# zhiqwang/yolort

Measured on NVIDIA H100. Metric: images/sec end-to-end (letterbox->NMS), higher is better.
Workload: dtype f16

## Files before the change

yolort_b200/_C.py:

```python
import ctypes
import itertools
import math
import os
from typing import Dict, List, Optional, Sequence, Tuple

import torch

_HERE = os.path.dirname(os.path.abspath(__file__))
LIB_PATH = os.environ.get("YB_LIB_PATH") or os.path.join(_HERE, "libyolort_b200.so")

YB_U8, YB_F16, YB_BF16, YB_F32, YB_F8E4M3 = 0, 1, 2, 3, 4
YB_LAYOUT_NCHW, YB_LAYOUT_S2D16 = 0, 1
YB_OP_CONV, YB_OP_SPP_POOL, YB_OP_UPSAMPLE2X, YB_OP_ATTENTION, YB_OP_DWCONV, YB_OP_SE, YB_OP_AVGPOOL = 0, 1, 2, 3, 4, 5, 6
YB_OP_QUANTIZE = 7
YB_ACT_NONE, YB_ACT_SILU, YB_ACT_HARDSWISH, YB_ACT_LEAKY01, YB_ACT_RELU = 0, 1, 2, 3, 4
YB_CONV_FORCE_IM2COL, YB_CONV_BAND_STEM, YB_CONV_FORCE_PLANES, YB_CONV_NO_NSPLIT, YB_CONV_ONE_CTA = 1, 2, 4, 8, 16
YB_CONV_NO_TAIL_SPLIT = 64
YB_CONV_PAIR_N64 = 128
YB_CONV_NO_TEAMS = 256
YB_CONV_E4M3_F16_OUT, YB_CONV_E4M3_BF16_OUT = 16, 32
YB_CONV_KERNEL_IM2COL, YB_CONV_KERNEL_PATCH, YB_CONV_KERNEL_E4M3 = 0, 1, 2
PATCH_TILINGS = {1: "classic", 2: "wrap", 3: "stride2"}
YB_MAX_LEVELS, YB_MAX_ANCHORS = 4, 4
NMS_TV_AUTO, NMS_EXACT_PER_CLASS, NMS_OFFSET_TRICK = 0, 1, 2
# ... 425 lines not shown
                                   ctypes.c_void_p]
    L.yb_kmeans_workspace_bytes.restype = ctypes.c_size_t
    L.yb_kmeans_workspace_bytes.argtypes = [ctypes.c_int64, ctypes.c_int, ctypes.c_int]
    L.yb_kmeans.argtypes = [ctypes.c_void_p, ctypes.c_int64, ctypes.c_int, ctypes.c_int, ctypes.c_void_p, ctypes.c_double,
                            ctypes.c_int, ctypes.c_void_p, ctypes.c_void_p, ctypes.c_void_p,
                            ctypes.POINTER(ctypes.c_int32), ctypes.c_void_p, ctypes.c_size_t, ctypes.c_void_p]
    L.yb_anchor_evolve.argtypes = [ctypes.c_void_p, ctypes.c_int64, ctypes.c_int, ctypes.c_void_p, ctypes.c_void_p,
                                   ctypes.c_int, ctypes.c_double, ctypes.c_int, ctypes.c_void_p, ctypes.c_void_p,
                                   ctypes.c_void_p, ctypes.c_void_p, ctypes.c_size_t, ctypes.c_void_p]
    L.yb_v5m_match_workspace_bytes.restype = ctypes.c_size_t
    L.yb_v5m_match_workspace_bytes.argtypes = [ctypes.c_int]
    L.yb_v5m_match.argtypes = [ctypes.c_int, ctypes.c_int] + [ctypes.c_void_p] * 5 + [ctypes.c_int] + \
        [ctypes.c_void_p] * 2 + [ctypes.c_int, ctypes.c_void_p, ctypes.c_int, ctypes.c_float, ctypes.c_float, ctypes.c_int] + \
        [ctypes.c_void_p] * 5 + [ctypes.c_size_t, ctypes.c_void_p]
    L.yb_v5m_ap_workspace_bytes.restype = ctypes.c_size_t
    L.yb_v5m_ap_workspace_bytes.argtypes = [ctypes.c_int64, ctypes.c_int]
    L.yb_v5m_ap.argtypes = [ctypes.c_void_p, ctypes.c_int64, ctypes.c_int, ctypes.c_int] + [ctypes.c_void_p] * 7 + \
        [ctypes.c_size_t, ctypes.c_void_p]
    _lib = L
    return L


def check(rc: int, what: str) -> None:
    if rc != 0:
        msg = lib().yb_last_error().decode("utf-8", "replace")
        raise NativeLibraryError(f"{what} failed (status {rc}): {msg}")


def dtype_code(dt: torch.dtype) -> int:
    try:
        return {torch.uint8: YB_U8, torch.float16: YB_F16, torch.bfloat16: YB_BF16, torch.float32: YB_F32,
                torch.float8_e4m3fn: YB_F8E4M3}[dt]
    except KeyError:
        raise NativeLibraryError(f"unsupported tensor dtype {dt}") from None


def current_stream_ptr(device: torch.device) -> int:
    return torch.cuda.current_stream(device).cuda_stream


class _NoGuard:
    def __enter__(self):
        return None

    def __exit__(self, *a):
        return False


_NO_GUARD = _NoGuard()


def device_guard(device: torch.device):
    idx = device.index if device.index is not None else torch.cuda.current_device()
    if torch.cuda.current_device() == idx:
        return _NO_GUARD
    return torch.cuda.device(idx)


def require_cuda(t: torch.Tensor, what: str) -> None:
    if not t.is_cuda:
        raise NativeLibraryError(
            f"{what}: tensor lives on {t.device}; the yolort_b200 path runs on sm_90a only (no CPU fallback)")


def letterbox_geometry(sizes: Sequence[Tuple[int, int]], min_size: float, max_size: float,
                       size_divisible: int = 32, fixed_shape: Optional[Tuple[int, int]] = None):
    n = len(sizes)
    hw = (ctypes.c_int32 * (2 * n))(*[int(v) for s in sizes for v in s])
    geoms = (LetterboxGeom * n)()
    bhw = (ctypes.c_int32 * 2)()
    fs = None
    if fixed_shape is not None:
        fs = (ctypes.c_int32 * 2)(int(fixed_shape[0]), int(fixed_shape[1]))
    check(lib().yb_letterbox_geometry(n, hw, float(min_size), float(max_size), int(size_divisible), fs, geoms, bhw),
          "yb_letterbox_geometry")
    return geoms, (int(bhw[0]), int(bhw[1]))


def scale_coords_params(Hb: int, Wb: int, h: int, w: int) -> Tuple[float, float, float]:
    out = (ctypes.c_float * 3)()
    check(lib().yb_scale_coords_params(int(Hb), int(Wb), int(h), int(w), out), "yb_scale_coords_params")
    return float(out[0]), float(out[1]), float(out[2])


_u8_lut: Dict[torch.device, torch.Tensor] = {}


def u8_lut(device: torch.device) -> torch.Tensor:
    t = _u8_lut.get(device)
    if t is None:
        t = (torch.arange(256, dtype=torch.uint8) / 255.0).to(torch.float32).to(device)
        _u8_lut[device] = t
    return t


YB_SRC_CHW, YB_SRC_HWC = 0, 1


def _is_hwc_view(im: torch.Tensor) -> bool:
    _, h, w = im.shape
    return tuple(im.stride()) == (1, 3 * w, 3) and (h > 1 or w > 1)


def letterbox(images: List[torch.Tensor], geoms, Hb: int, Wb: int, fill: float, out: torch.Tensor,
              layout: int) -> torch.Tensor:
    n = len(images)
    dev = out.device
    require_cuda(out, "letterbox")
    src_dtype = images[0].dtype
    ptrs = (ctypes.c_void_p * n)()
    keep = []
    for im in images:
        require_cuda(im, "letterbox")
        if im.dtype != src_dtype:
            raise NativeLibraryError("letterbox: all images of a batch must share a dtype")
        if im.dim() != 3 or im.shape[0] != 3:
            raise ValueError(f"images is expected to be a list of 3d tensors of shape [C, H, W], but got '{im.shape}'.")
    hwc = all(_is_hwc_view(im) for im in images)
    for i, im in enumerate(images):
        if not hwc:
            im = im.contiguous()
        keep.append(im)
        ptrs[i] = im.data_ptr()
    lut = u8_lut(dev) if src_dtype == torch.uint8 else None
    with device_guard(dev):
        check(lib().yb_letterbox_strided(n, ptrs, dtype_code(src_dtype), YB_SRC_HWC if hwc else YB_SRC_CHW, geoms,
                                         int(Hb), int(Wb), float(fill), lut.data_ptr() if lut is not None else None,
                                         out.data_ptr(), dtype_code(out.dtype), int(layout), current_stream_ptr(dev)),
              "yb_letterbox")
    stream = torch.cuda.current_stream(dev)
    seen = set()
    for im in keep:
        key = im.untyped_storage().data_ptr()
        if key not in seen:
            seen.add(key)
            im.record_stream(stream)
    return out


def conv_chain_supported(op: "OpDesc") -> bool:
    return bool(lib().yb_conv_chain_supported(ctypes.byref(op)))


def conv_config(op: "OpDesc") -> dict:
    info = ConvInfo()
    check(lib().yb_conv_config(ctypes.byref(op), ctypes.byref(info)), "yb_conv_config")
    patch = info.kernel == YB_CONV_KERNEL_PATCH
    cfg = {k: int(getattr(info, k)) for k in ("block_n", "n_tiles", "weights_resident", "tiles_per_pass", "slots", "ring",
                                               "store_cols", "smem_bytes", "grid", "chained", "resident_ctas", "m_tiles",
                                               "work_items", "tail_n", "tail_tiles", "tail_split")}
    cfg["patch_kernel"] = int(patch)
    cfg["e4m3_kernel"] = int(info.kernel == YB_CONV_KERNEL_E4M3)
    cfg["store_bufs" if patch else "epilogue_groups"] = int(info.store_bufs if patch else info.groups)
    cfg["layout"] = f"{info.resident_ctas}x{info.groups}"
    cfg["consumer_groups"] = int(info.groups)
    cfg["ctas_per_sm"] = 2 if cfg["layout"] == "2x2" else 1
    if patch:
        cfg["patch_tiling"] = PATCH_TILINGS[info.tiling]
    return cfg


class Plan:

    def __init__(self, ops: Sequence[OpDesc], device: torch.device):
        arr = (OpDesc * len(ops))(*ops)
        handle = ctypes.c_void_p()
        with torch.cuda.device(device):
            check(lib().yb_plan_create(arr, len(ops), ctypes.byref(handle)), "yb_plan_create")
        self._h = handle
        self.device = device
        self.n_ops = len(ops)

    def run(self, first: int = 0, count: Optional[int] = None) -> None:
        if count is None:
            count = self.n_ops - first
        with device_guard(self.device):
            check(lib().yb_plan_run_range(self._h, first, count, current_stream_ptr(self.device)), "yb_plan_run")

    def __del__(self):
        h = getattr(self, "_h", None)
        if h is not None and _lib is not None:
            _lib.yb_plan_destroy(h)
            self._h = None


class _NmsArena:

    def __init__(self):
        self.ws: Optional[torch.Tensor] = None
        self.cap_per_image = 16384


_arenas: Dict[torch.device, _NmsArena] = {}


def _level_struct(t: torch.Tensor, layout: str, n_anchors: int, n_outputs: int, stride_px: float,
                  anchors: Sequence[float]) -> HeadLevel:
    lv = HeadLevel()
    lv.logits = t.data_ptr()
    lv.dtype = dtype_code(t.dtype)
    if layout == "nahwk":
        if t.dim() != 5 or t.shape[1] != n_anchors or t.shape[4] != n_outputs or not t.is_contiguous():
            raise NativeLibraryError(f"decode_nms: expected contiguous [N,{n_anchors},H,W,{n_outputs}], got {tuple(t.shape)}")
        N, A, H, W, K = t.shape
        lv.H, lv.W = H, W
        lv.stride_n, lv.stride_a, lv.stride_y, lv.stride_x = A * H * W * K, H * W * K, W * K, K
    elif layout == "nhwc":
        if t.dim() != 4 or t.shape[3] < n_anchors * n_outputs or not t.is_contiguous():
            raise NativeLibraryError(f"decode_nms: expected contiguous [N,H,W,>={n_anchors * n_outputs}], got {tuple(t.shape)}")
        N, H, W, C = t.shape
        lv.H, lv.W = H, W
        lv.stride_n, lv.stride_a, lv.stride_y, lv.stride_x = H * W * C, n_outputs, W * C, C
    else:
        raise NativeLibraryError(f"unknown head layout {layout!r}")
    lv.stride_px = float(stride_px)
    for i, v in enumerate(anchors):
        lv.anchors_px[i] = float(v)
    return lv


def decode_nms_padded(head_outputs: List[torch.Tensor], layout: str, strides: Sequence[float],
                      anchors_px: Sequence[Sequence[float]], num_classes: int, score_thresh: float,
                      nms_thresh: float, detections_per_img: int, semantics: int = NMS_TV_AUTO,
                      rescale: Optional[torch.Tensor] = None, stage_hook=None):
    t0 = head_outputs[0]
    require_cuda(t0, "decode_nms")
    dev = t0.device
    n_images = int(t0.shape[0])
    n_levels = len(head_outputs)
    n_anchors = len(anchors_px[0]) // 2
    if n_levels > YB_MAX_LEVELS or n_anchors > YB_MAX_ANCHORS:
        raise NativeLibraryError("decode_nms: too many levels/anchors")
    arena = _arenas.setdefault(dev, _NmsArena())
    levels = (HeadLevel * n_levels)(*[
        _level_struct(t, layout, n_anchors, num_classes + 5, strides[i], anchors_px[i])
        for i, t in enumerate(head_outputs)])
    D = int(detections_per_img)
    boxes = torch.empty((n_images, D, 4), dtype=torch.float32, device=dev)
    scores = torch.empty((n_images, D), dtype=torch.float32, device=dev)
    labels = torch.empty((n_images, D), dtype=torch.int64, device=dev)
    counts = torch.empty((n_images,), dtype=torch.int32, device=dev)
    status = torch.empty((4,), dtype=torch.int64, device=dev)
    p = NmsParams(n_images, n_levels, n_anchors, int(num_classes), float(score_thresh), float(nms_thresh), D,
                  int(semantics), int(arena.cap_per_image) * n_images)
    need = lib().yb_decode_nms_workspace_bytes(ctypes.byref(p), levels)
    if arena.ws is None or arena.ws.numel() < need or arena.ws.device != dev:
        arena.ws = torch.empty((need,), dtype=torch.uint8, device=dev)
    with device_guard(dev):
        if stage_hook is None:
            check(lib().yb_decode_nms(ctypes.byref(p), levels, rescale.data_ptr() if rescale is not None else None,
                                      boxes.data_ptr(), scores.data_ptr(), labels.data_ptr(), counts.data_ptr(),
                                      status.data_ptr(), arena.ws.data_ptr(), arena.ws.numel(), current_stream_ptr(dev)),
                  "yb_decode_nms")
        else:
            st = current_stream_ptr(dev)
            check(lib().yb_nms_begin(ctypes.byref(p), levels, status.data_ptr(), arena.ws.data_ptr(), arena.ws.numel(), st),
                  "yb_nms_begin")
            stage_hook("begin")
            check(lib().yb_decode_candidates(ctypes.byref(p), levels, arena.ws.data_ptr(), arena.ws.numel(), st),
                  "yb_decode_candidates")
            stage_hook("decode")
            check(lib().yb_nms_finish(ctypes.byref(p), levels, rescale.data_ptr() if rescale is not None else None,
                                      boxes.data_ptr(), scores.data_ptr(), labels.data_ptr(), counts.data_ptr(),
                                      status.data_ptr(), arena.ws.data_ptr(), arena.ws.numel(), st), "yb_nms_finish")
            stage_hook("nms")
    arena.debug_offset = lib().yb_decode_nms_debug_offset(ctypes.byref(p), levels)
    return boxes, scores, labels, counts, status


def decode_dense(head_outputs: List[torch.Tensor], layout: str, strides: Sequence[float],
                 anchors_px: Sequence[Sequence[float]], num_classes: int):
    t0 = head_outputs[0]
    require_cuda(t0, "decode_dense")
    dev = t0.device
    n_images, n_levels = int(t0.shape[0]), len(head_outputs)
    n_anchors = len(anchors_px[0]) // 2
    if n_levels > YB_MAX_LEVELS or n_anchors > YB_MAX_ANCHORS:
        raise NativeLibraryError("decode_dense: too many levels/anchors")
    levels = (HeadLevel * n_levels)(*[
        _level_struct(t, layout, n_anchors, num_classes + 5, strides[i], anchors_px[i])
        for i, t in enumerate(head_outputs)])
    total = sum(n_anchors * int(lv.H) * int(lv.W) for lv in levels)
    boxes = torch.empty((n_images, total, 4), dtype=torch.float32, device=dev)
    scores = torch.empty((n_images, total, int(num_classes)), dtype=torch.float32, device=dev)
    p = NmsParams(n_images, n_levels, n_anchors, int(num_classes), 0.0, 0.0, 1, 0, 0)
    with device_guard(dev):
        check(lib().yb_decode_dense(ctypes.byref(p), levels, boxes.data_ptr(), scores.data_ptr(), current_stream_ptr(dev)),
              "yb_decode_dense")
    return boxes, scores


def nms_phase_clocks(device) -> list:
    arena = _arenas[torch.device(device)]
    off = arena.debug_offset
    return arena.ws[off: off + 128].view(torch.int64)[4:10].cpu().tolist()


def decode_nms(head_outputs: List[torch.Tensor], layout: str, strides, anchors_px, score_thresh: float,
               nms_thresh: float, detections_per_img: int, semantics: int = NMS_TV_AUTO,
               rescale: Optional[torch.Tensor] = None, num_classes: Optional[int] = None) -> List[Dict[str, torch.Tensor]]:
    if num_classes is None:
        t0 = head_outputs[0]
        num_classes = int(t0.shape[4]) - 5 if layout == "nahwk" else None
        if num_classes is None:
            raise NativeLibraryError("decode_nms: num_classes is required for the nhwc layout")
    dev = head_outputs[0].device
    while True:
# ... 647 lines not shown
```

yolort_b200/csrc/conv_sm90.cu:

```cuda
#include <cstdlib>

#include "common.cuh"
#include "conv_sm90.h"
#include "conv_epilogue.cuh"
#include "conv_chain.cuh"
#include "decode_common.cuh"

namespace yb {

namespace {

constexpr int kMaxStages = 12;
__host__ __device__ constexpr int tile_rows(int groups) { return 64 * groups; }
__host__ __device__ constexpr int cta_threads(int groups) { return 128 * (1 + groups); }
__host__ __device__ constexpr int stage_buf_bytes(int groups) { return tile_rows(groups) * 128; }
constexpr int kStageBufs = 2;
constexpr int kMaxBlockN = 256;
constexpr size_t kSmemBudget = 216 * 1024;
constexpr size_t kStaticSmem = (2 * kMaxStages + 2) * 8 + 2 * kMaxBlockN * 4;
constexpr uint32_t kConsumerBar = 1;

struct ConvKernelParams {
  int M, block_n, block_k;
  int ksize, chunks, num_k_iters;
  int mode;
  int HoWo, Wo, stride, pad;
  int stages;
  int kpg;
  int b_resident;
  uint32_t b_res_bytes;
  int n_tiles, num_tiles;
  int full_tiles, split, num_tasks;
  int ctas;
  int groups;
  int store_cols;
  int bias_len;
  int kk_last;
  uint32_t a_stage_bytes, b_stage_bytes;
  const float* bias;
  EpilogueParams ep;
  ChainParams ch;
  int decode_on;
  int dec_H, dec_W;
  yb_head_decode dec;
};

template <int kGroups>
__device__ __forceinline__ void consumer_sync() { named_bar_sync(kConsumerBar, 128 * kGroups); }

struct ConvTask {
  int m_tile, n_tile, piece, split;
};
template <bool kSplits>
__device__ __forceinline__ ConvTask conv_task(const ConvKernelParams& p, int t) {
  ConvTask k;
  int tile = t;
  k.piece = 0;
  k.split = 1;
  if (kSplits && t >= p.full_tiles) {
    const int u = t - p.full_tiles;
    const int q = u / p.n_tiles;
    tile = p.full_tiles + (q / p.split) * p.n_tiles + (u - q * p.n_tiles);
    k.piece = q % p.split;
    k.split = p.split;
  }
  k.m_tile = tile / p.n_tiles;
  k.n_tile = tile - k.m_tile * p.n_tiles;
  return k;
}

template <bool kBf16, int kW>
__device__ __forceinline__ int stage_mmas(float* acc, const ConvKernelParams& p, uint32_t a_lo0, uint32_t a_step16,
                                          uint32_t b_lo0, uint32_t b_step16, uint64_t ab_hi, int cnt, int ch, int kk,
                                          bool first) {
  for (int j = 0; j < cnt; ++j) {
    const int kc = ch == p.chunks - 1 ? p.kk_last : kk;
    for (int k = 0; k < kc; ++k)
      wgmma_mma<kBf16, kW>(acc, desc_lohi(a_lo0 + j * a_step16 + 2 * k, ab_hi), desc_lohi(b_lo0 + j * b_step16 + 2 * k, ab_hi),
                           !first || (j | k) != 0);
    if (++ch == p.chunks) ch = 0;
  }
  return ch;
}

template <int kN>
__device__ __forceinline__ void decode_fragment(const yb_head_decode& D, const float* acc, const float* s_bias,
                                                const FragRows& fr, int dec_H, int dec_W, float* head, uint32_t wg_bar,
                                                int lane) {
  constexpr int kMaxA = 4;
  const int K = D.n_classes + 5;
  const int q2 = 2 * (lane & 3);
#pragma unroll
  for (int j = 0; j < kN / 8; ++j) {
    {
#pragma unroll
      for (int i = 0; i < 4; ++i) {
        const int col = 8 * j + q2 + (i & 1);
        const int a = col / K, r = col - a * K;
        if (a < D.n_anchors && r < 5) head[fr.loc[i >> 1] * 20 + a * 5 + r] = acc[4 * j + i] + s_bias[col];
      }
    }
  }
  named_bar_sync(wg_bar, 128);
  float obj[2][kMaxA];
  bool pass[2][kMaxA];
  uint32_t emitted[2] = {0u, 0u};
#pragma unroll
  for (int rr = 0; rr < 2; ++rr) {
#pragma unroll
    for (int a = 0; a < kMaxA; ++a) {
      obj[rr][a] = a < D.n_anchors ? sigmoidf_ref(head[fr.loc[rr] * 20 + a * 5 + 4]) : 0.f;
      pass[rr][a] = a < D.n_anchors && fr.ok[rr] && obj[rr][a] > D.score_thresh;
    }
  }
  int n_img[2], py[2], px[2];
  const int hw = dec_H * dec_W;
#pragma unroll
  for (int rr = 0; rr < 2; ++rr) {
    n_img[rr] = static_cast<int>(fr.row[rr] / hw);
    const int rem = static_cast<int>(fr.row[rr] - static_cast<long long>(n_img[rr]) * hw);
    py[rr] = rem / dec_W;
    px[rr] = rem - py[rr] * dec_W;
  }
  const bool any_pass = pass[0][0] || pass[0][1] || pass[0][2] || pass[0][3] || pass[1][0] || pass[1][1] ||
                        pass[1][2] || pass[1][3];
  if (any_pass) {
#pragma unroll
    for (int j = 0; j < kN / 8; ++j) {
      {
#pragma unroll
        for (int i = 0; i < 4; ++i) {
          const int rr = i >> 1;
          const int col = 8 * j + q2 + (i & 1);
          const int a = col / K, r = col - a * K;
          const bool pa = a == 0 ? pass[rr][0] : (a == 1 ? pass[rr][1] : (a == 2 ? pass[rr][2] : (a == 3 && pass[rr][3])));
          if (pa && r >= 5) {
            const float oa = a == 0 ? obj[rr][0] : (a == 1 ? obj[rr][1] : (a == 2 ? obj[rr][2] : obj[rr][3]));
            const float score = __fmul_rn(sigmoidf_ref(acc[4 * j + i] + s_bias[col]), oa);
            if (score > D.score_thresh) {
              const int anchor_flat = D.level_start + (a * dec_H + py[rr]) * dec_W + px[rr];
              emit_candidate(D.keys, D.img_count, D.cap_per_image, n_img[rr], anchor_flat, D.n_classes, r - 5, score);
              emitted[rr] |= 1u << a;
            }
          }
        }
      }
    }
  }
#pragma unroll
  for (int rr = 0; rr < 2; ++rr) {
    emitted[rr] |= __shfl_xor_sync(0xffffffffu, emitted[rr], 1);
    emitted[rr] |= __shfl_xor_sync(0xffffffffu, emitted[rr], 2);
    if ((lane & 3) == 0 && emitted[rr]) {
      const float* h = head + fr.loc[rr] * 20;
      for (int a = 0; a < D.n_anchors; ++a) {
        if (!((emitted[rr] >> a) & 1u)) continue;
        const int anchor_flat = D.level_start + (a * dec_H + py[rr]) * dec_W + px[rr];
        const float4 b = decode_box(sigmoidf_ref(h[a * 5 + 0]), sigmoidf_ref(h[a * 5 + 1]), sigmoidf_ref(h[a * 5 + 2]),
                                    sigmoidf_ref(h[a * 5 + 3]), px[rr], py[rr], D.stride_px, D.anchors_px[2 * a],
                                    D.anchors_px[2 * a + 1]);
        reinterpret_cast<float4*>(D.boxes)[static_cast<long long>(n_img[rr]) * D.anchors_per_image + anchor_flat] = b;
        atomicMax(&D.img_maxc[n_img[rr]], float_to_ordered_int(fmaxf(fmaxf(b.x, b.y), fmaxf(b.z, b.w))));
      }
    }
  }
  named_bar_sync(wg_bar, 128);
}

template <bool kBf16, int kN, bool kDecode, int kN2, int kCtas, int kGroups = 2>
__global__ void __launch_bounds__(cta_threads(kGroups), kCtas)
conv_wgmma_kernel(const __grid_constant__ CUtensorMap tmap_a, const __grid_constant__ CUtensorMap tmap_b,
                  const __grid_constant__ CUtensorMap tmap_out, const __grid_constant__ CUtensorMap tmap_w2,
                  const __grid_constant__ CUtensorMap tmap_out2, const __grid_constant__ CUtensorMap tmap_a64,
                  const __grid_constant__ CUtensorMap tmap_out64, const ConvKernelParams p) {
  static_assert(kGroups == 2 || (kGroups == 1 && kCtas == 2 && !kDecode), "one consumer warpgroup: two CTAs, no decode");
  constexpr bool kChain = kN2 != 0;
  constexpr int kAcc = (kN > kN2 ? kN : kN2) / 2;
  constexpr int kBlockM = tile_rows(kGroups);
  constexpr int kStageBufBytes = stage_buf_bytes(kGroups);
  constexpr bool kSplits = !kDecode && !kChain && kN == 128;
  constexpr bool kRowHalves = kSplits && kGroups == 2;
  extern __shared__ uint8_t smem_raw[];
  __shared__ __align__(8) uint64_t full_bar[kMaxStages];
  __shared__ __align__(8) uint64_t empty_bar[kMaxStages];
  __shared__ __align__(8) uint64_t b_full;
  __shared__ __align__(8) uint64_t w2_full;
  __shared__ __align__(16) float s_bias[kMaxBlockN];
// ... 276 lines not shown
    }
    mbar_init(&b_full, 1);
    mbar_init(&w2_full, 1);
    mbar_fence_init();
  }
  __syncthreads();

  if (threadIdx.x == 0) {
    const uint32_t b_bytes = p.block_n * p.block_k * 2;
    mbar_expect_tx(&b_full, p.num_k_iters * b_bytes);
    for (int it = 0; it < p.num_k_iters; ++it) tma_load_2d(&tmap_b, &b_full, b_res + it * p.b_stage_bytes, it * p.block_k, 0);
    tma_prefetch_desc(&tmap_w2);
    tma_prefetch_desc(&tmap_out2);
    mbar_expect_tx(&w2_full, p.ch.w2_chunks * p.ch.n2 * p.ch.w2_row_bytes);
    for (int j = 0; j < p.ch.w2_chunks; ++j)
      tma_load_2d(&tmap_w2, &w2_full, w2_res + j * p.ch.w2_sub_bytes, j * (p.ch.w2_row_bytes >> 1), 0);
  }
  asm volatile("griddepcontrol.wait;" ::: "memory");
  asm volatile("griddepcontrol.launch_dependents;" ::: "memory");
  if (warp < 4) {
    asm volatile("setmaxnreg.dec.sync.aligned.u32 24;\n" ::: "memory");
    if (warp != 0) return;
    const uint32_t a_bytes = p.a_stage_bytes;
    int kit0 = 0, kit1 = 0;
    for (int t = blockIdx.x, k = 0; t < p.num_tiles; t += gridDim.x, ++k) {
      const int r = k & 1;
      const int m0 = t * 128;
      int kit = r ? kit1 : kit0;
      for (int it = 0; it < p.num_k_iters; ++it, ++kit) {
        const int s = kit % p.stages;
        mbar_wait(&empty_bar[r][s], ((kit / p.stages) & 1) ^ 1);
        if (YB_ELECT()) {
          mbar_expect_tx(&full_bar[r][s], a_bytes);
          tma_load_2d(&tmap_a, &full_bar[r][s], tiles + r * ring_bytes + s * a_bytes, it * p.block_k, m0);
        }
      }
      (r ? kit1 : kit0) = kit;
    }
    return;
  }
  asm volatile("setmaxnreg.inc.sync.aligned.u32 112;\n" ::: "memory");

  const int cw = (warp >> 2) - 1;
  const int team = cw >> 1, half = cw & 1;
  const int wq = warp & 3;
  const int ctid = threadIdx.x - 128;
  const bool issuer = (ctid & 255) == 0;
  const bool wg_leader = (threadIdx.x & 127) == 0;
  const uint32_t team_bar = kTeamBar0 + team;
  FragRows fr;
  fr.loc[0] = half * 64 + wq * 16 + (lane >> 2);
  fr.loc[1] = fr.loc[0] + 8;
  uint8_t* team_staging = staging + static_cast<size_t>(team) * kStageBufs * kStageBufBytes;
  uint8_t* ring = tiles + team * ring_bytes;
  float acc[kN / 2];

  for (int i = ctid; i < kN; i += 512) s_bias[i] = (i < p.bias_len) ? __ldg(p.bias + i) : 0.f;
  for (int i = ctid; i < kN2; i += 512) s_bias2[i] = (i < p.ch.bias2_len) ? __ldg(p.ch.bias2 + i) : 0.f;
  named_bar_sync(kConsumerBar, 512);
  mbar_wait(&b_full, 0);
  mbar_wait(&w2_full, 0);

  int kit = 0;
  for (int t = blockIdx.x + team * gridDim.x; t < p.num_tiles; t += 2 * gridDim.x) {
    const int m0 = t * 128;
    {
      const uint32_t ab_hi = desc_hi(128, 8 * 128);
      const uint32_t a_wg16 = (64 * 128 * half) >> 4;
      const uint32_t b_lo0 = smem_lo16(b_res);
      const uint32_t b_step16 = p.b_stage_bytes >> 4;
#pragma unroll
      for (int i = 0; i < kN / 2; ++i) acc[i] = 0.f;
      int prev_s = -1;
      for (int it = 0; it < p.num_k_iters; ++it, ++kit) {
        const int s = kit % p.stages;
        mbar_wait(&full_bar[team][s], (kit / p.stages) & 1);
        const uint32_t a_lo = smem_lo16(ring + s * p.a_stage_bytes) + a_wg16;
        const uint32_t b_lo = b_lo0 + it * b_step16;
        wgmma_fence();
#pragma unroll
        for (int k = 0; k < 4; ++k)
          wgmma_mma<kBf16, kN>(acc, desc_lohi(a_lo + 2 * k, ab_hi), desc_lohi(b_lo + 2 * k, ab_hi), it != 0 || k != 0);
        wgmma_commit();
        wgmma_wait<1>();
        if (prev_s >= 0 && wg_leader) mbar_arrive(&empty_bar[team][prev_s]);
        prev_s = s;
      }
      wgmma_wait<0>();
      fence_acc<kN / 2>(acc);
      if (wg_leader) mbar_arrive(&empty_bar[team][prev_s]);
    }

#pragma unroll
    for (int rr = 0; rr < 2; ++rr) {
      fr.row[rr] = static_cast<long long>(m0) + fr.loc[rr];
      fr.ok[rr] = fr.row[rr] < p.M;
    }
    if (issuer) tma_store_wait_read<0>();
    named_bar_sync(team_bar, 256);
#pragma unroll
    for (int c0 = 0; c0 < kN; c0 += 64) {
      uint8_t* buf = team_staging + (c0 / 64) * kStageBufBytes;
      epilogue_box<kBf16, kN>(p.ep, acc, c0, 64, s_bias, fr, 0, buf, lane);
      fence_proxy_async_smem();
      named_bar_sync(team_bar, 256);
      if (issuer) {
        if (p.ch.store_first && c0 < p.ep.Cout) tma_store_2d(&tmap_out, buf, c0, m0);
        tma_store_commit();
      }
    }
    {
      const uint32_t a2_hi = desc_hi(128, 8 * 128);
      const uint32_t w2_hi = desc_hi(p.ch.w2_row_bytes, 8 * p.ch.w2_row_bytes);
      const uint32_t stag_lo = smem_lo16(team_staging) + ((64 * half * 128) >> 4);
      const uint32_t w2_lo0 = smem_lo16(w2_res);
      const uint32_t w2_step16 = p.ch.w2_sub_bytes >> 4;
      wgmma_fence();
      if (p.ch.own_chunks == 2) {
#pragma unroll
        for (int j = 0; j < 2; ++j)
#pragma unroll
          for (int k = 0; k < 4; ++k)
            wgmma_mma<kBf16, kN2>(acc, desc_lohi(stag_lo + j * (kStageBufBytes >> 4) + 2 * k, a2_hi),
                                  desc_lohi(w2_lo0 + j * w2_step16 + 2 * k, w2_hi), (j | k) != 0);
      } else {
#pragma unroll
        for (int k = 0; k < 4; ++k)
          wgmma_mma<kBf16, kN2>(acc, desc_lohi(stag_lo + 2 * k, a2_hi), desc_lohi(w2_lo0 + 2 * k, w2_hi), k != 0);
      }
      wgmma_commit();
      wgmma_wait<0>();
      fence_acc<kN2 / 2>(acc);
    }
    if (issuer) tma_store_wait_read<0>();
    named_bar_sync(team_bar, 256);
    EpilogueParams ep2 = p.ch.ep2;
    ep2.residual = nullptr;
#pragma unroll
    for (int c0 = 0; c0 < kN2; c0 += 64) {
      uint8_t* buf = team_staging + ((c0 / 64) & 1) * kStageBufBytes;
      epilogue_box<kBf16, kN2>(ep2, acc, c0, 64, s_bias2, fr, 0, buf, lane);
      fence_proxy_async_smem();
      if (issuer) tma_store_wait_read<0>();
      named_bar_sync(team_bar, 256);
      if (issuer) {
        if (c0 < p.ch.ep2.Cout) tma_store_2d(&tmap_out2, buf, c0, m0);
        tma_store_commit();
      }
    }
  }
  if (issuer) tma_store_wait_all<0>();
}

using ConvKernelFn =void (*)(const CUtensorMap, const CUtensorMap, const CUtensorMap, const CUtensorMap, const CUtensorMap,
                              const CUtensorMap, const CUtensorMap, const ConvKernelParams);

template <bool kBf16>
ConvKernelFn select_conv_kernel_t(const ConvKernelParams& kp) {
  if (kp.groups == 4)
    return kp.block_n == 128 && kp.ch.n2 == 64 ? conv_wgmma_team_kernel<kBf16, 128, 64> : nullptr;
  if (kp.groups == 1) {
    if (kp.ctas != 2 || kp.decode_on || kp.ch.on) return nullptr;
    return kp.block_n == 128 ? conv_wgmma_kernel<kBf16, 128, false, 0, 2, 1> : nullptr;
  }
  if (kp.ctas == 2) {
    if (kp.decode_on) return nullptr;
    if (kp.ch.on) {
      if (kp.block_n != 64) return nullptr;
      return kp.ch.n2 == 32 ? conv_wgmma_kernel<kBf16, 64, false, 32, 2>
                            : (kp.ch.n2 == 64 ? conv_wgmma_kernel<kBf16, 64, false, 64, 2> : nullptr);
    }
    switch (kp.block_n) {
      case 16: return conv_wgmma_kernel<kBf16, 16, false, 0, 2>;
      case 32: return conv_wgmma_kernel<kBf16, 32, false, 0, 2>;
      case 64: return conv_wgmma_kernel<kBf16, 64, false, 0, 2>;
      default: return nullptr;
    }
  }
  if (kp.decode_on) return conv_wgmma_kernel<kBf16, 256, true, 0, 1>;
  if (kp.ch.on) {
    if (kp.block_n == 64)
      return kp.ch.n2 == 32 ? conv_wgmma_kernel<kBf16, 64, false, 32, 1>
                            : (kp.ch.n2 == 64 ? conv_wgmma_kernel<kBf16, 64, false, 64, 1> : conv_wgmma_kernel<kBf16, 64, false, 128, 1>);
    return kp.ch.n2 == 32 ? conv_wgmma_kernel<kBf16, 128, false, 32, 1>
                          : (kp.ch.n2 == 64 ? conv_wgmma_kernel<kBf16, 128, false, 64, 1> : conv_wgmma_kernel<kBf16, 128, false, 128, 1>);
  }
  switch (kp.block_n) {
    case 16: return conv_wgmma_kernel<kBf16, 16, false, 0, 1>;
    case 32: return conv_wgmma_kernel<kBf16, 32, false, 0, 1>;
    case 64: return conv_wgmma_kernel<kBf16, 64, false, 0, 1>;
    case 128: return conv_wgmma_kernel<kBf16, 128, false, 0, 1>;
    default: return conv_wgmma_kernel<kBf16, 256, false, 0, 1>;
  }
}
ConvKernelFn select_conv_kernel(const ConvKernelParams& kp) {
  return kp.ep.is_bf16 ? select_conv_kernel_t<true>(kp) : select_conv_kernel_t<false>(kp);
}

}

static int conv_plan(const yb_op_desc& d, int ctas, int groups, ConvKernelParams& kp, dim3& grid, size_t& smem_bytes);
static void conv_team_plan(ConvKernelParams& kp, size_t& smem_bytes);

int conv_validate(const yb_op_desc& d) {
  YB_REQUIRE(d.dtype == YB_F16 || d.dtype == YB_BF16, "conv: dtype must be f16 or bf16");
  YB_REQUIRE((d.reserved & ~(31 | YB_CONV_NO_TAIL_SPLIT | YB_CONV_PAIR_N64 | YB_CONV_NO_TEAMS)) == 0,
             "conv: reserved bits 5 and 9 and up must be zero, got 0x%x",
             d.reserved);
  YB_REQUIRE(d.ksize >= 1 && d.ksize <= 7 && d.stride >= 1 && d.stride <= 2, "conv: ksize/stride");
  YB_REQUIRE(d.act >= YB_ACT_NONE && d.act <= YB_ACT_RELU, "conv: unknown activation %d", d.act);
  YB_REQUIRE(d.Cin % 8 == 0 && d.in_cstride % 8 == 0 && d.in_cstride >= d.Cin,
             "conv: Cin/in_cstride must be multiples of 8 (16-byte TMA granularity), got %d/%d", d.Cin,
             d.in_cstride);
  YB_REQUIRE(d.Cout % 8 == 0 && d.out_cstride % 8 == 0 && d.out_cstride >= d.Cout,
             "conv: Cout/out_cstride must be multiples of 8, got %d/%d", d.Cout, d.out_cstride);
  YB_REQUIRE(d.Cin_pad % 16 == 0 && d.Cin_pad >= d.Cin, "conv: Cin_pad must be a multiple of 16");
  YB_REQUIRE(d.Cout_pad % 16 == 0 && d.Cout_pad >= d.Cout, "conv: Cout_pad must be a multiple of 16");
  YB_REQUIRE((reinterpret_cast<uintptr_t>(d.in) & 15) == 0 && (reinterpret_cast<uintptr_t>(d.out) & 15) == 0 &&
                 (reinterpret_cast<uintptr_t>(d.weight) & 15) == 0,
             "conv: tensors must be 16-byte aligned");
  YB_REQUIRE(d.residual == nullptr ||
                 ((reinterpret_cast<uintptr_t>(d.residual) & 15) == 0 && d.res_cstride % 8 == 0),
             "conv: residual alignment");
  int M;
  return conv_rows(d, "conv", &M);
}

static int conv_configure(const yb_op_desc& d, ConvKernelParams& kp, dim3& grid, size_t& smem_bytes) {
  const int rc = conv_validate(d);
  if (rc != YB_OK) return rc;
  YB_REQUIRE(!(d.reserved & YB_CONV_BAND_STEM),
             "conv: banded stem weights (reserved bit 1) need the halo-patch kernel, which this %dx%d map does not qualify for",
             d.H, d.W);
  if (!(d.reserved & YB_CONV_ONE_CTA) &&
      (conv_plan(d, 2, 2, kp, grid, smem_bytes) == YB_OK || conv_plan(d, 2, 1, kp, grid, smem_bytes) == YB_OK))
    return YB_OK;
  const int rc1 = conv_plan(d, 1, 2, kp, grid, smem_bytes);
  if (rc1 == YB_OK && !(d.reserved & (YB_CONV_ONE_CTA | YB_CONV_NO_TEAMS | YB_CONV_PAIR_N64)))
    conv_team_plan(kp, smem_bytes);
  return rc1;
}

static void conv_team_plan(ConvKernelParams& kp, size_t& smem_bytes) {
  if (!(kp.ctas == 1 && kp.groups == 2 && kp.mode == 0 && kp.ch.on && !kp.decode_on && kp.b_resident &&
        kp.n_tiles == 1 && kp.block_n == 128 && kp.ch.n2 == 64 && kp.block_k == 64 && kp.kk_last == 4 &&
        kp.ch.ksteps == 4 && kp.num_tiles >= kTeamMinTilesPerSm * num_sms()))
    return;
  const size_t fixed = kp.b_res_bytes + 2 * kStageBufs * static_cast<size_t>(stage_buf_bytes(2)) +
                       static_cast<size_t>(kp.ch.w2_chunks) * kp.ch.w2_sub_bytes + 1024;
  if (fixed >= kTeamSmemBudget) return;
  int stages = static_cast<int>((kTeamSmemBudget - fixed) / (2 * static_cast<size_t>(kp.a_stage_bytes)));
  if (stages < 2) return;
  if (stages > kTeamMaxStages) stages = kTeamMaxStages;
  kp.groups = 4;
  kp.kpg = 1;
  kp.stages = stages;
  smem_bytes = fixed + 2 * static_cast<size_t>(stages) * kp.a_stage_bytes;
}

static int conv_plan(const yb_op_desc& d, int ctas, int groups, ConvKernelParams& kp, dim3& grid, size_t& smem_bytes) {
  const int Ho = d.Ho, Wo = d.Wo;
  const size_t budget = ctas == 2 ? smem_per_sm() / 2 - kSmemReservedPerCta - kStaticSmem : kSmemBudget;
  const int block_m = tile_rows(groups);
  kp = ConvKernelParams();
  kp.ctas = ctas;
  kp.groups = groups;
  kp.M = static_cast<int>(static_cast<long long>(d.N) * Ho * Wo);
  kp.ep.Cout = d.Cout;
  const int m_tiles = (kp.M + block_m - 1) / block_m;
  const int sms = num_sms();
  const int m_tiles128 = (kp.M + tile_rows(2) - 1) / tile_rows(2);
  int block_n = conv_block_n(d.Cout, m_tiles128, d.chain != nullptr);
  if (groups == 1) {
    if (block_n != 256 || d.chain != nullptr || m_tiles128 < 3 * sms) return YB_ERR_INVALID;
    block_n = 128;
  }
  if (groups == 2 && ctas == 1 && block_n == 256 && d.chain == nullptr && d.decode == nullptr &&
      !(d.reserved & (YB_CONV_NO_TAIL_SPLIT | YB_CONV_ONE_CTA)) && static_cast<size_t>(d.ksize) * d.ksize * d.Cin_pad * 256 * 2 > 80 * 1024 &&
      m_tiles > sms && m_tiles < 4 * sms && m_tiles % sms != 0) {
    const int n128 = (d.Cout + 127) / 128, r128 = (m_tiles * n128) % sms;
    if (sms % n128 == 0 && r128 > 0 && 2 * r128 <= sms) block_n = 128;
  }
  int n_tiles = (d.Cout + block_n - 1) / block_n;
  YB_REQUIRE(mma_n(block_n) == block_n && block_n <= kMaxBlockN, "conv: N tile %d is not a wgmma N", block_n);
  kp.block_n = block_n;
  kp.n_tiles = n_tiles;
  kp.num_tiles = m_tiles * n_tiles;
  kp.block_k = (d.Cin_pad % 64 == 0) ? 64 : ((d.Cin_pad % 32 == 0) ? 32 : 16);
  kp.ksize = d.ksize;
  kp.chunks = d.Cin_pad / kp.block_k;
  kp.num_k_iters = d.ksize * d.ksize * kp.chunks;
  kp.mode = (d.ksize == 1 && d.stride == 1 && d.pad == 0) ? 0 : 1;
  kp.HoWo = Ho * Wo;
  kp.Wo = Wo;
  kp.stride = d.stride;
  kp.pad = d.pad;
  kp.decode_on = 0;
  if (d.decode != nullptr) {
    const yb_head_decode& dd = *d.decode;
    const int width = dd.n_anchors * (dd.n_classes + 5);
    if (!(dd.n_anchors > 0 && dd.n_anchors <= 4 && width <= kMaxBlockN && width <= d.Cout_pad && d.ksize == 1 &&
          dd.keys && dd.boxes && dd.img_count && dd.img_maxc)) {
      set_error("conv: fused decode needs a 1x1 head with n_anchors*(n_classes+5) <= %d and a candidate arena", kMaxBlockN);
      return YB_ERR_INVALID;
    }
    n_tiles = 1;
    block_n = mma_n(d.Cout);
    YB_REQUIRE(block_n == 256, "conv: the fused decode is built for heads of 129-256 columns, got %d", d.Cout);
    kp.block_n = block_n;
    kp.n_tiles = 1;
    kp.num_tiles = m_tiles;
    kp.decode_on = 1;
    kp.dec = dd;
    kp.dec_H = Ho;
    kp.dec_W = Wo;
  }
  kp.store_cols = (block_n % 64 == 0) ? 64 : ((block_n % 32 == 0) ? 32 : 16);
  kp.bias_len = d.Cout_pad;
  kp.kk_last = (d.Cin - (kp.chunks - 1) * kp.block_k + 15) / 16;
  if (kp.kk_last < 1) kp.kk_last = 1;
  if (kp.kk_last > (kp.block_k >> 4)) kp.kk_last = kp.block_k >> 4;
  kp.a_stage_bytes = block_m * kp.block_k * 2;
  kp.b_stage_bytes = (static_cast<uint32_t>(kp.block_n * kp.block_k * 2) + 1023u) & ~1023u;
  kp.ch.on = 0;
  size_t chain_bytes = 0;
  if (d.chain != nullptr) {
    YB_REQUIRE(kp.store_cols == 64, "conv: a chained tail needs 64-column output boxes (Cout %% 64 == 0), got Cout=%d", d.Cout);
    const char* why = chain_setup(d, kp.block_n, kp.n_tiles, kp.store_cols, false, &kp.ch);
    YB_REQUIRE(why == nullptr, "conv: chained tail not supported here: %s", why);
    const int s2 = chain_store2_cols(kp.ch.n2);
    YB_REQUIRE(s2 == 64 || s2 == 32, "conv: the tail's Cout_pad must be a multiple of 32, got %d", kp.ch.n2);
    YB_REQUIRE((kp.block_n == 64 || kp.block_n == 128) && kp.ch.n2 <= 128,
               "conv: chained tails are built for N tiles of 64 / 128 and tails of at most 128 columns (block_n=%d, n2=%d)",
               kp.block_n, kp.ch.n2);
    chain_bytes = static_cast<size_t>(kp.ch.w2_chunks) * kp.ch.w2_sub_bytes;
  }
  const size_t fixed = static_cast<size_t>(kStageBufs) * stage_buf_bytes(groups) + 1024 + chain_bytes;
  const bool fixed_n = n_tiles == 1 || (groups == 1 && (2 * sms) % n_tiles == 0);
  KPipeline pipe;
  const int rc = size_k_pipeline(budget, fixed, kp.a_stage_bytes, kp.b_stage_bytes, kp.num_k_iters, fixed_n, kMaxStages,
                                 "conv", kp.block_n, &pipe);
  if (rc != YB_OK) return rc;
  kp.b_resident = pipe.b_resident;
  kp.b_res_bytes = pipe.b_res_bytes;
  kp.kpg = pipe.kpg;
  kp.stages = pipe.stages;
  kp.ep.is_bf16 = d.dtype == YB_BF16;
  kp.ep.act = d.act;
  kp.bias = d.bias;
  kp.ep.residual = d.residual;
  kp.ep.res_cstride = d.res_cstride;
  if (ctas == 2 && (select_conv_kernel(kp) == nullptr || kp.num_tiles < 2 * sms)) return YB_ERR_INVALID;
  if (groups == 1) {
    ConvKernelParams two = kp;
    two.groups = 2;
    if (!kp.b_resident || select_conv_kernel(two) != nullptr) return YB_ERR_INVALID;
  }
  const int max_grid = ctas * sms;
  grid = dim3(kp.num_tiles < max_grid ? kp.num_tiles : max_grid, 1, 1);
  const int G = static_cast<int>(grid.x);
  const int r = kp.num_tiles % G;
  kp.split = !(d.reserved & YB_CONV_NO_TAIL_SPLIT) && !kp.decode_on && !kp.ch.on && kp.block_n == 128 &&
                     G % kp.n_tiles == 0 && r > 0 && 2 * r <= G ? 2 : 1;
  kp.full_tiles = kp.split > 1 ? kp.num_tiles - r : kp.num_tiles;
  kp.num_tasks = kp.full_tiles + (kp.num_tiles - kp.full_tiles) * kp.split;
  smem_bytes = pipe.smem;
  return YB_OK;
}

int im2col_conv_config(const yb_op_desc& d, yb_conv_info* info) {
  ConvKernelParams kp;
  dim3 grid;
  size_t smem = 0;
  const int rc = conv_configure(d, kp, grid, smem);
  if (rc == YB_OK && info) {
    info->kernel = YB_CONV_KERNEL_IM2COL;
    info->block_n = kp.block_n;
    info->n_tiles = kp.n_tiles;
    info->weights_resident = kp.b_resident;
    info->tiles_per_pass = 1;
    info->slots = kp.stages;
    info->ring = kp.kpg;
    info->store_cols = kp.store_cols;
    info->store_bufs = kStageBufs;
    info->groups = kp.groups;
    info->resident_ctas = kp.ctas;
    info->chained = kp.ch.on;
    info->smem_bytes = static_cast<int>(smem);
    info->grid = static_cast<int>(grid.x);
    info->tiling = YB_CONV_TILING_ROWS;
    info->m_tiles = kp.num_tiles / kp.n_tiles;
    info->work_items = kp.num_tiles;
    info->tail_n = kp.ch.n2;
    info->tail_tiles = kp.split > 1 ? kp.num_tiles - kp.full_tiles : 0;
    info->tail_split = kp.split;
  }
  return rc;
}

struct Im2colConvOp final : ConvOp {
  CUtensorMap tmap_a, tmap_b, tmap_out, tmap_w2, tmap_out2, tmap_a64, tmap_out64;
  ConvKernelParams kp;
  ConvKernelFn fn = nullptr;
  dim3 grid;
  size_t smem_bytes;
  int launch(cudaStream_t stream) const override {
    YB_CHECK_CUDA(launch_pdl(fn, grid, dim3(cta_threads(kp.groups)), smem_bytes, stream, tmap_a, tmap_b, tmap_out, tmap_w2,
                             tmap_out2, tmap_a64, tmap_out64, kp));
    return YB_OK;
  }
};

int im2col_conv_create(const yb_op_desc& d, ConvOp** out) {
  Im2colConvOp* op = new Im2colConvOp();
  ConvKernelParams& kp = op->kp;
  int rc = conv_configure(d, kp, op->grid, op->smem_bytes);
  const bool teams = kp.groups == 4;
  const uint32_t block_m = tile_rows(teams ? 2 : kp.groups);
  const CUtensorMapDataType dt = kp.ep.is_bf16 ? CU_TENSOR_MAP_DATA_TYPE_BFLOAT16 : CU_TENSOR_MAP_DATA_TYPE_FLOAT16;
  if (rc == YB_OK)
    rc = kp.mode == 0 ? tmap_matrix(&op->tmap_a, "conv input", dt, d.in, d.Cin, kp.M, d.in_cstride, kp.block_k, block_m,
                                    CU_TENSOR_MAP_L2_PROMOTION_L2_128B)
                      : tmap_im2col(&op->tmap_a, "conv input", dt, d, kp.block_k, block_m);
  const int ktot = d.ksize * d.ksize * d.Cin_pad;
  if (rc == YB_OK)
    rc = tmap_matrix(&op->tmap_b, "conv weights", dt, d.weight, ktot, d.Cout_pad, ktot, kp.block_k, kp.block_n,
                     CU_TENSOR_MAP_L2_PROMOTION_L2_256B);
  if (rc == YB_OK)
    rc = tmap_matrix(&op->tmap_out, "conv output", dt, d.out, d.Cout, kp.M, d.out_cstride, kp.store_cols, block_m,
                     CU_TENSOR_MAP_L2_PROMOTION_NONE);
  op->tmap_w2 = op->tmap_b;
  op->tmap_out2 = op->tmap_out;
  op->tmap_a64 = op->tmap_a;
  op->tmap_out64 = op->tmap_out;
  if (rc == YB_OK && kp.split > 1 && kp.groups == 2) {
    rc = kp.mode == 0 ? tmap_matrix(&op->tmap_a64, "conv input (tail halves)", dt, d.in, d.Cin, kp.M, d.in_cstride,
                                    kp.block_k, 64, CU_TENSOR_MAP_L2_PROMOTION_L2_128B)
                      : tmap_im2col(&op->tmap_a64, "conv input (tail halves)", dt, d, kp.block_k, 64);
    if (rc == YB_OK)
      rc = tmap_matrix(&op->tmap_out64, "conv output (tail halves)", dt, d.out, d.Cout, kp.M, d.out_cstride, kp.store_cols,
                       64, CU_TENSOR_MAP_L2_PROMOTION_NONE);
  }
  if (rc == YB_OK && kp.ch.on) {
    const yb_conv_chain& c = *d.chain;
    rc = tmap_matrix(&op->tmap_w2, "conv chained tail weights", dt, c.weight, c.K_pad, c.Cout_pad, c.K_pad,
                     kp.ch.w2_row_bytes / 2, kp.ch.n2, CU_TENSOR_MAP_L2_PROMOTION_L2_256B);
    if (rc == YB_OK)
      rc = tmap_matrix(&op->tmap_out2, "conv chained tail output", dt, c.out, c.Cout, kp.M, c.out_cstride,
                       chain_store2_cols(kp.ch.n2), block_m, CU_TENSOR_MAP_L2_PROMOTION_NONE);
  }
  if (rc == YB_OK) {
    op->fn = select_conv_kernel(kp);
    rc = set_smem_attributes(reinterpret_cast<const void*>(op->fn), teams ? kTeamSmemBudget : kSmemBudget, kp.ctas,
                             op->smem_bytes, cta_threads(kp.groups), "conv");
    if (rc == YB_OK && teams) {
      int per_sm = 0;
      const cudaError_t e =
          cudaOccupancyMaxActiveBlocksPerMultiprocessor(&per_sm, op->fn, cta_threads(kp.groups), op->smem_bytes);
      if (e != cudaSuccess) {
        set_error("conv: cudaOccupancyMaxActiveBlocksPerMultiprocessor failed: %s", cudaGetErrorString(e));
        rc = YB_ERR_CUDA;
      } else if (per_sm < 1) {
        set_error("conv: the two-team CTA (%d threads, %zu bytes of shared memory) does not fit on an SM",
                  cta_threads(kp.groups), op->smem_bytes);
        rc = YB_ERR_INVALID;
      }
    }
  }
  if (rc != YB_OK) {
    delete op;
    return rc;
  }
  *out = op;
  return YB_OK;
}

}
```

Before: 8950.

## Add quad-warpgroup conv kernel sharing weight tiles across paired M tiles

Adds a conv kernel in which one CTA runs four consumer warpgroups as two teams. Each team computes its own 128-row M tile, and both teams share a single B (weight) stage loaded once per k-step. The planner picks this kernel for large non-resident, unchained, non-residual convs with block_n 128, in place of the two-group single-CTA plan. The aim is to halve weight-tile TMA traffic and fill SMs better on big layers. The cost is fewer pipeline stages per tile and tail imbalance when m_tiles is odd.

```diff
diff --git a/yolort_b200/_C.py b/yolort_b200/_C.py
--- a/yolort_b200/_C.py
+++ b/yolort_b200/_C.py
@@ -601,7 +601,8 @@
     cfg["patch_kernel"] = int(patch)
     cfg["e4m3_kernel"] = int(info.kernel == YB_CONV_KERNEL_E4M3)
     cfg["store_bufs" if patch else "epilogue_groups"] = int(info.store_bufs if patch else info.groups)
-    cfg["layout"] = f"{info.resident_ctas}x{info.groups}"
+    pairs = not patch and info.groups == 4 and info.tiles_per_pass == 2
+    cfg["layout"] = f"{info.resident_ctas}x{info.groups}" + ("x2" if pairs else "")
     cfg["consumer_groups"] = int(info.groups)
     cfg["ctas_per_sm"] = 2 if cfg["layout"] == "2x2" else 1
     if patch:
diff --git a/yolort_b200/csrc/conv_sm90.cu b/yolort_b200/csrc/conv_sm90.cu
--- a/yolort_b200/csrc/conv_sm90.cu
+++ b/yolort_b200/csrc/conv_sm90.cu
@@ -33,6 +33,7 @@
   int full_tiles, split, num_tasks;
   int ctas;
   int groups;
+  int pair;
   int store_cols;
   int bias_len;
   int kk_last;
@@ -615,11 +616,167 @@
   if (issuer) tma_store_wait_all<0>();
 }
 
+constexpr size_t kQuadStaticSmem = 2 * kMaxStages * 8 + 128 * 4;
+constexpr size_t kQuadSmemBudget = 227 * 1024 - kQuadStaticSmem;
+constexpr int kQuadMinMTiles = 100;
+constexpr int kQuadWideMTiles = 400;
+
+template <bool kBf16>
+__global__ void __launch_bounds__(kTeamThreads, 1)
+conv_wgmma_quad_kernel(const __grid_constant__ CUtensorMap tmap_a, const __grid_constant__ CUtensorMap tmap_b,
+                       const __grid_constant__ CUtensorMap tmap_out, const __grid_constant__ CUtensorMap,
+                       const __grid_constant__ CUtensorMap, const __grid_constant__ CUtensorMap,
+                       const __grid_constant__ CUtensorMap, const ConvKernelParams p) {
+  constexpr int kN = 128;
+  constexpr int kStageBufBytes = stage_buf_bytes(2);
+  extern __shared__ uint8_t smem_raw[];
+  __shared__ __align__(8) uint64_t full_bar[kMaxStages];
+  __shared__ __align__(8) uint64_t empty_bar[kMaxStages];
+  __shared__ __align__(16) float s_bias[kN];
+
+  uint8_t* tiles = reinterpret_cast<uint8_t*>(
+      (reinterpret_cast<uintptr_t>(smem_raw) + 1023) & ~static_cast<uintptr_t>(1023));
+  const uint32_t stage_bytes = 2 * p.a_stage_bytes + p.b_stage_bytes;
+  uint8_t* staging = tiles + static_cast<size_t>(p.stages) * stage_bytes;
+
+  const int warp = threadIdx.x >> 5;
+  const int lane = threadIdx.x & 31;
+
+  if (threadIdx.x == 0) {
+    tma_prefetch_desc(&tmap_a);
+    tma_prefetch_desc(&tmap_b);
+    tma_prefetch_desc(&tmap_out);
+    for (int s = 0; s < p.stages; ++s) {
+      mbar_init(&full_bar[s], 1);
+      mbar_init(&empty_bar[s], 4);
+    }
+    mbar_fence_init();
+  }
+  __syncthreads();
+  asm volatile("griddepcontrol.wait;" ::: "memory");
+  asm volatile("griddepcontrol.launch_dependents;" ::: "memory");
+  if (warp < 4) {
+    asm volatile("setmaxnreg.dec.sync.aligned.u32 24;\n" ::: "memory");
+    if (warp != 0) return;
+    const uint32_t a_bytes = p.a_stage_bytes, b_bytes = p.block_n * p.block_k * 2;
+    const int m_tiles = p.num_tiles / p.n_tiles;
+    int kit = 0;
+    for (int t = blockIdx.x; t < p.num_tasks; t += gridDim.x) {
+      const int q = t / p.n_tiles;
+      const int n0 = (t - q * p.n_tiles) * p.block_n;
+      const int cnt = min(2, m_tiles - 2 * q);
+      for (int it = 0; it < p.num_k_iters; ++it, ++kit) {
+        const int s = kit % p.stages;
+        mbar_wait(&empty_bar[s], ((kit / p.stages) & 1) ^ 1);
+        uint8_t* a_dst = tiles + s * stage_bytes;
+        if (YB_ELECT()) {
+          mbar_expect_tx(&full_bar[s], cnt * a_bytes + b_bytes);
+          const int tap = it / p.chunks;
+          const int chunk = it - tap * p.chunks;
+          for (int j = 0; j < cnt; ++j) {
+            const int m0 = (2 * q + j) * 128;
+            if (p.mode == 0) {
+              tma_load_2d(&tmap_a, &full_bar[s], a_dst + j * a_bytes, chunk * p.block_k, m0);
+            } else {
+              const int cn = m0 / p.HoWo;
+              const int rem = m0 - cn * p.HoWo;
+              const int ho = rem / p.Wo;
+              const int wo = rem - ho * p.Wo;
+              const int r = tap / p.ksize;
+              const int sx = tap - r * p.ksize;
+              tma_load_im2col_4d(&tmap_a, &full_bar[s], a_dst + j * a_bytes, chunk * p.block_k, wo * p.stride - p.pad,
+                                 ho * p.stride - p.pad, cn, static_cast<uint16_t>(sx), static_cast<uint16_t>(r));
+            }
+          }
+          tma_load_2d(&tmap_b, &full_bar[s], a_dst + 2 * a_bytes, it * p.block_k, n0);
+        }
+      }
+    }
+    return;
+  }
+  asm volatile("setmaxnreg.inc.sync.aligned.u32 112;\n" ::: "memory");
+
+  const int cw = (warp >> 2) - 1;
+  const int team = cw >> 1, half = cw & 1;
+  const int wq = warp & 3;
+  const int ctid = threadIdx.x - 128;
+  const bool issuer = (ctid & 255) == 0;
+  const bool wg_leader = (threadIdx.x & 127) == 0;
+  const uint32_t team_bar = kTeamBar0 + team;
+  FragRows fr;
+  fr.loc[0] = half * 64 + wq * 16 + (lane >> 2);
+  fr.loc[1] = fr.loc[0] + 8;
+  uint8_t* team_staging = staging + static_cast<size_t>(team) * kStageBufs * kStageBufBytes;
+  EpilogueParams ep = p.ep;
+  ep.residual = nullptr;
+  float acc[kN / 2];
+
+  const int n0 = (blockIdx.x % p.n_tiles) * kN;
+  for (int i = ctid; i < kN; i += 512) s_bias[i] = (n0 + i < p.bias_len) ? __ldg(p.bias + n0 + i) : 0.f;
+  named_bar_sync(kConsumerBar, 512);
+
+  const int m_tiles = p.num_tiles / p.n_tiles;
+  int kit = 0, store_idx = 0;
+  for (int t = blockIdx.x; t < p.num_tasks; t += gridDim.x) {
+    const int mt = 2 * (t / p.n_tiles) + team;
+    const bool active = mt < m_tiles;
+    const int m0 = mt * 128;
+    {
+      const uint32_t ab_hi = desc_hi(128, 8 * 128);
+      const uint32_t a_off16 = (p.a_stage_bytes * team + 64 * 128 * half) >> 4;
+      const uint32_t b_off16 = (2 * p.a_stage_bytes) >> 4;
+      const uint32_t tiles_lo = smem_lo16(tiles);
+      const uint32_t stage16 = stage_bytes >> 4;
+#pragma unroll
+      for (int i = 0; i < kN / 2; ++i) acc[i] = 0.f;
+      int prev_s = -1;
+      for (int it = 0; it < p.num_k_iters; ++it, ++kit) {
+        const int s = kit % p.stages;
+        mbar_wait(&full_bar[s], (kit / p.stages) & 1);
+        const uint32_t st_lo = tiles_lo + s * stage16;
+        wgmma_fence();
+#pragma unroll
+        for (int k = 0; k < 4; ++k)
+          wgmma_mma<kBf16, kN>(acc, desc_lohi(st_lo + a_off16 + 2 * k, ab_hi), desc_lohi(st_lo + b_off16 + 2 * k, ab_hi),
+                               it != 0 || k != 0);
+        wgmma_commit();
+        wgmma_wait<1>();
+        if (prev_s >= 0 && wg_leader) mbar_arrive(&empty_bar[prev_s]);
+        prev_s = s;
+      }
+      wgmma_wait<0>();
+      fence_acc<kN / 2>(acc);
+      if (wg_leader) mbar_arrive(&empty_bar[prev_s]);
+    }
+
+#pragma unroll
+    for (int rr = 0; rr < 2; ++rr) {
+      fr.row[rr] = static_cast<long long>(m0) + fr.loc[rr];
+      fr.ok[rr] = active && fr.row[rr] < p.M;
+    }
+#pragma unroll
+    for (int c0 = 0; c0 < kN; c0 += 64, ++store_idx) {
+      uint8_t* buf = team_staging + (store_idx & 1) * kStageBufBytes;
+      epilogue_box<kBf16, kN>(ep, acc, c0, 64, s_bias, fr, n0, buf, lane);
+      fence_proxy_async_smem();
+      if (issuer) tma_store_wait_read<0>();
+      named_bar_sync(team_bar, 256);
+      if (issuer) {
+        if (active && n0 + c0 < p.ep.Cout) tma_store_2d(&tmap_out, buf, n0 + c0, m0);
+        tma_store_commit();
+      }
+    }
+  }
+  if (issuer) tma_store_wait_all<0>();
+}
+
 using ConvKernelFn =void (*)(const CUtensorMap, const CUtensorMap, const CUtensorMap, const CUtensorMap, const CUtensorMap,
                               const CUtensorMap, const CUtensorMap, const ConvKernelParams);
 
 template <bool kBf16>
 ConvKernelFn select_conv_kernel_t(const ConvKernelParams& kp) {
+  if (kp.groups == 4 && kp.pair == 2)
+    return kp.block_n == 128 && !kp.ch.on ? conv_wgmma_quad_kernel<kBf16> : nullptr;
   if (kp.groups == 4)
     return kp.block_n == 128 && kp.ch.n2 == 64 ? conv_wgmma_team_kernel<kBf16, 128, 64> : nullptr;
   if (kp.groups == 1) {
@@ -664,6 +821,7 @@
 
 static int conv_plan(const yb_op_desc& d, int ctas, int groups, ConvKernelParams& kp, dim3& grid, size_t& smem_bytes);
 static void conv_team_plan(ConvKernelParams& kp, size_t& smem_bytes);
+static void conv_quad_plan(ConvKernelParams& kp, dim3& grid, size_t& smem_bytes);
 
 int conv_validate(const yb_op_desc& d) {
   YB_REQUIRE(d.dtype == YB_F16 || d.dtype == YB_BF16, "conv: dtype must be f16 or bf16");
@@ -701,6 +859,8 @@
   const int rc1 = conv_plan(d, 1, 2, kp, grid, smem_bytes);
   if (rc1 == YB_OK && !(d.reserved & (YB_CONV_ONE_CTA | YB_CONV_NO_TEAMS | YB_CONV_PAIR_N64)))
     conv_team_plan(kp, smem_bytes);
+  if (rc1 == YB_OK && !(d.reserved & (YB_CONV_ONE_CTA | YB_CONV_PAIR_N64 | YB_CONV_NO_TAIL_SPLIT)))
+    conv_quad_plan(kp, grid, smem_bytes);
   return rc1;
 }
 
@@ -721,6 +881,33 @@
   smem_bytes = fixed + 2 * static_cast<size_t>(stages) * kp.a_stage_bytes;
 }
 
+static void conv_quad_plan(ConvKernelParams& kp, dim3& grid, size_t& smem_bytes) {
+  if (!(kp.ctas == 1 && kp.groups == 2 && !kp.b_resident && kp.block_n == 128 && !kp.ch.on && !kp.decode_on &&
+        kp.ep.residual == nullptr && kp.block_k == 64 && kp.kk_last == 4))
+    return;
+  const int sms = num_sms();
+  const int m_tiles = kp.num_tiles / kp.n_tiles;
+  const int T = (m_tiles + 1) / 2 * kp.n_tiles;
+  const int G = T < sms ? T : sms;
+  if (G % kp.n_tiles != 0 || m_tiles < kQuadMinMTiles ||
+      !(m_tiles <= sms || kp.n_tiles >= 3 || m_tiles >= kQuadWideMTiles))
+    return;
+  const uint32_t stage_bytes = 2 * kp.a_stage_bytes + kp.b_stage_bytes;
+  const size_t fixed = 2 * kStageBufs * static_cast<size_t>(stage_buf_bytes(2)) + 1024;
+  int stages = static_cast<int>((kQuadSmemBudget - fixed) / stage_bytes);
+  if (stages < 2) return;
+  if (stages > kMaxStages) stages = kMaxStages;
+  kp.groups = 4;
+  kp.pair = 2;
+  kp.kpg = 1;
+  kp.stages = stages;
+  kp.split = 1;
+  kp.full_tiles = kp.num_tiles;
+  kp.num_tasks = T;
+  grid = dim3(G, 1, 1);
+  smem_bytes = fixed + static_cast<size_t>(stages) * stage_bytes;
+}
+
 static int conv_plan(const yb_op_desc& d, int ctas, int groups, ConvKernelParams& kp, dim3& grid, size_t& smem_bytes) {
   const int Ho = d.Ho, Wo = d.Wo;
   const size_t budget = ctas == 2 ? smem_per_sm() / 2 - kSmemReservedPerCta - kStaticSmem : kSmemBudget;
@@ -728,6 +915,7 @@
   kp = ConvKernelParams();
   kp.ctas = ctas;
   kp.groups = groups;
+  kp.pair = 1;
   kp.M = static_cast<int>(static_cast<long long>(d.N) * Ho * Wo);
   kp.ep.Cout = d.Cout;
   const int m_tiles = (kp.M + block_m - 1) / block_m;
@@ -841,7 +1029,7 @@
     info->block_n = kp.block_n;
     info->n_tiles = kp.n_tiles;
     info->weights_resident = kp.b_resident;
-    info->tiles_per_pass = 1;
+    info->tiles_per_pass = kp.pair;
     info->slots = kp.stages;
     info->ring = kp.kpg;
     info->store_cols = kp.store_cols;
@@ -914,8 +1102,9 @@
   }
   if (rc == YB_OK) {
     op->fn = select_conv_kernel(kp);
-    rc = set_smem_attributes(reinterpret_cast<const void*>(op->fn), teams ? kTeamSmemBudget : kSmemBudget, kp.ctas,
-                             op->smem_bytes, cta_threads(kp.groups), "conv");
+    const size_t budget = kp.pair == 2 ? kQuadSmemBudget : (teams ? kTeamSmemBudget : kSmemBudget);
+    rc = set_smem_attributes(reinterpret_cast<const void*>(op->fn), budget, kp.ctas, op->smem_bytes,
+                             cta_threads(kp.groups), "conv");
     if (rc == YB_OK && teams) {
       int per_sm = 0;
       const cudaError_t e =
@@ -924,7 +1113,7 @@
         set_error("conv: cudaOccupancyMaxActiveBlocksPerMultiprocessor failed: %s", cudaGetErrorString(e));
         rc = YB_ERR_CUDA;
       } else if (per_sm < 1) {
-        set_error("conv: the two-team CTA (%d threads, %zu bytes of shared memory) does not fit on an SM",
+        set_error("conv: the four-warpgroup CTA (%d threads, %zu bytes of shared memory) does not fit on an SM",
                   cta_threads(kp.groups), op->smem_bytes);
         rc = YB_ERR_INVALID;
       }
```

New measurement: 9514 (median of 6 runs). 1.06x the previous value.
